# vislearn/esac

Hardware: NVIDIA H100
Metric: pose hypotheses scored/sec (640x480, 256 hyp x E experts) (higher is better)
Workload: dtype f32 (scoring) / f64 (P3P, refinement)

## Files before the change

esac_b200/csrc/capi.cu:

```cuda
#include <cuda_runtime.h>
#include <dlfcn.h>
#include <stdarg.h>
#include <stdio.h>
#include <stdlib.h>
#include <string.h>

#include <algorithm>
#include <exception>
#include <new>
#include <string>
#include <vector>
#include <thread>
#include <chrono>

#include "../../include/esac_b200.h"
#include "../../include/esac_b200_testhooks.h"
#include "esac_internal.h"
#include "esac_p3p_fast.cuh"
#include "esac_rng.cuh"

using namespace esacb200;

namespace {

// ... 225 lines not shown
    if (is_device_ptr(assign)) {
        pl.d_assign = (const long long*)assign;
        pl.assign_stride = stride;
    } else {
        std::vector<long long> tmp((size_t)P.M);
        for (int h = 0; h < P.M; ++h) tmp[h] = (long long)assign[(long long)h * stride];
        CK(abuf.ensure((size_t)P.M * 8));
        CK(cudaMemcpyAsync(abuf.p, tmp.data(), (size_t)P.M * 8, cudaMemcpyHostToDevice, copy_stream));
        pl.d_assign = abuf.as<long long>();
        pl.assign_stride = 1;
    }
    return 0;
}

void plan_launch(esacb200_ctx* ctx, Plan& pl) {
    const Problem& P = pl.P;
    int ppt = 8, hc = 64;
    const int want = 2 * 2 * ctx->sm_count;
    auto items = [&](int ppt_, int hc_) {
        int T = (P.N + score_tile_pixels(ppt_) - 1) / score_tile_pixels(ppt_);
        int nch = (P.M + hc_ - 1) / hc_ + (P.E > 1 ? P.E / 2 : 0);
        return (long long)T * nch;
    };
    if (items(8, 64) < want) { ppt = 4; hc = 32; }
    if (ppt == 4 && items(4, 32) < want) { ppt = 2; hc = 16; }
    if (ctx->score_ppt_opt == 2 || ctx->score_ppt_opt == 4 || ctx->score_ppt_opt == 8) ppt = ctx->score_ppt_opt;
    if (ctx->score_hc_opt > 0) hc = ctx->score_hc_opt < 64 ? ctx->score_hc_opt : 64;
    pl.ppt = ppt;
    pl.hc = hc;
    pl.T = (P.N + score_tile_pixels(ppt) - 1) / score_tile_pixels(ppt);
    const int max_chunks = (P.M + hc - 1) / hc + P.E;
    long long it = (long long)pl.T * max_chunks;
    pl.grid = (int)(it < 2ll * ctx->sm_count ? it : 2ll * ctx->sm_count);
    const int need_align = ppt >= 4 ? 4 : 2;
    pl.vec_ok = (P.N % need_align == 0) && (((uintptr_t)pl.d_coords) % (need_align * 4) == 0);
}

int plan_and_prep(esacb200_ctx* ctx, Plan& pl) {
    const Problem& P = pl.P;
    plan_launch(ctx, pl);
    CK(ctx->assign32.ensure((size_t)P.M * 4));
    CK(ctx->counts.ensure((size_t)P.E * 4));
    CK(ctx->offsets.ensure((size_t)(P.E + 1) * 4));
    CK(ctx->perm.ensure((size_t)P.M * 4));
    CK(ctx->slot_of.ensure((size_t)P.M * 4));
    CK(ctx->chunks.ensure((size_t)(P.M + P.E) * sizeof(ChunkDesc)));
    CK(ctx->scalars.ensure(S_COUNT * 4));
    CK(ctx->centres.ensure((size_t)P.E * 3 * 4));
    CK(ctx->poses.ensure((size_t)P.M * sizeof(Pose)));
    CK(ctx->poses_ref.ensure((size_t)P.M * sizeof(Pose)));
    CK(ctx->cells.ensure((size_t)P.M * 8 * 4));
    CK(ctx->tries.ensure((size_t)P.M * 4));
    CK(ctx->posepk.ensure((size_t)P.M * sizeof(PosePk)));
    CK(ctx->part.ensure((size_t)P.M * pl.T * 4));
    CK(ctx->scores.ensure((size_t)P.M * 8));
    CK(ctx->probs.ensure((size_t)P.M * 8));
    CK(ctx->stats.ensure(8 * 8));
    CK(ctx->contrib.ensure((size_t)P.M * 4));
    CK(ctx->out17.ensure(32 * 4));
    int* sc = ctx->scalars.as<int>();
    launch_prep(pl.d_coords, pl.d_assign, pl.assign_stride, P, pl.hc, ctx->assign32.as<int>(), ctx->counts.as<int>(),
                ctx->offsets.as<int>(), ctx->perm.as<int>(), ctx->slot_of.as<int>(), ctx->chunks.as<ChunkDesc>(),
                sc + S_NCHUNKS, sc + S_WORK, ctx->centres.as<float>(), sc + S_FLAGS, pl.split_e ? 1 : 3, ctx->stream);
    ctx->st.kernel_launches += 1;
    mark(ctx, EV_PREP);
    return 0;
}

int stage_inputs(esacb200_ctx* ctx, Plan& pl, const float* coords, const int64_t* assign, int64_t stride, bool allow_split = false) {
    int rc = upload_inputs(ctx, pl, coords, assign, stride, ctx->coords, ctx->assign64, ctx->stream, allow_split);
    if (rc) return rc;
    mark(ctx, EV_H2D);
    return plan_and_prep(ctx, pl);
}

constexpr int kSampleCap = 1 << 19;
constexpr int kSampleCapAcc = 1 << 15;

struct SampleSizes {
    int G, Mg;
    size_t per_group_ints, int_bytes, per_group_bytes, surv_bytes;
};
SampleSizes sample_sizes(const esacb200_ctx* ctx, const Plan& pl) {
    const Problem& P = pl.P;
    SampleSizes z;
    int G = pl.split_e ? 2 : ((ctx->sample_groups > 1 && ctx->aux_stream && P.M >= 64 && (P.N >= 65536 || P.M >= 1024)) ? ctx->sample_groups : 1);
    if (G > 2 && (!ctx->aux_more[0] || !ctx->aux_more[1] || P.M < 512)) G = 2;
    z.G = G;
    z.Mg = pl.split_e ? P.M : (P.M + G - 1) / G;
    z.per_group_ints = (size_t)2 * z.Mg + 8;
    z.int_bytes = ((size_t)P.M * 4 + G * z.per_group_ints) * 4 + 8;
    z.per_group_bytes = (size_t)kSampleCap * sizeof(int2) + (size_t)kSampleCapAcc * sizeof(Accepted);
    z.surv_bytes = G * z.per_group_bytes;
    return z;
}

int run_sample(esacb200_ctx* ctx, const Plan& pl, uint64_t seed) {
    const Problem& P = pl.P;
    const int cap = kSampleCap;
    const int cap_acc = kSampleCapAcc;
    const SampleSizes z = sample_sizes(ctx, pl);
    const int G = z.G, Mg = z.Mg;
    const size_t per_group_ints = z.per_group_ints, per_group_bytes = z.per_group_bytes;
    CK(ctx->smp_int.ensure(z.int_bytes));
    CK(ctx->smp_surv.ensure(z.surv_bytes));
    SampleState st[4];
    int* b = ctx->smp_int.as<int>() + 2 * (size_t)P.M;
    for (int g = 0; g < G; ++g) {
        st[g].best = ctx->smp_int.as<unsigned long long>();
        st[g].base = b;
        st[g].ovf = b + P.M;
        st[g].list = b + 2 * (size_t)P.M + g * per_group_ints;
        st[g].counters = st[g].list + 2 * (size_t)Mg;
        char* sb = (char*)ctx->smp_surv.p + g * per_group_bytes;
        st[g].surv = (int2*)sb;
        st[g].stage = (Accepted*)(sb + (size_t)cap * sizeof(int2));
        st[g].cap = cap;
        st[g].cap_acc = cap_acc;
        st[g].M = Mg;
    }
    CK(ctx->coords4.ensure((size_t)P.E * P.N * sizeof(float4)));
    unsigned long long* trace = nullptr;
    if (ctx->sample_trace) {
        CK(ctx->smp_trace.ensure(512 * 8));
        CK(cudaMemsetAsync(ctx->smp_trace.p, 0, 512 * 8, ctx->stream));
        trace = ctx->smp_trace.as<unsigned long long>();
        launch_trace_init(trace, 256, ctx->stream);
    }
    const cudaStream_t lane_streams[4] = {ctx->stream, ctx->aux_stream, ctx->aux_more[0], ctx->aux_more[1]};
    const cudaEvent_t lane_joins[4] = {nullptr, ctx->ev_join, ctx->ev_join_more[0], ctx->ev_join_more[1]};
    ctx->st.kernel_launches += launch_sample(pl.d_coords, ctx->coords4.as<float4>(), ctx->assign32.as<int>(), P, seed, ctx->max_tries,
                                             ctx->inj_M ? ctx->inject.as<int>() : nullptr, ctx->inj_T, st, G, ctx->sm_count,
                                             ctx->sample_prefilter, ctx->hyp_offset, ctx->hyp_stride, ctx->poses.as<Pose>(), ctx->cells.as<int>(),
                                             ctx->tries.as<int>(), lane_streams, ctx->ev_fork, lane_joins,
                                             pl.split_e, ctx->perm.as<int>(), ctx->offsets.as<int>(), ctx->ev_copied,
                                             ctx->sample_span0, ctx->sample_window, ctx->sample_waves, trace, ctx->sample_tail_boost);
    CK(cudaGetLastError());
    ctx->smp_groups_last = G;
    ctx->smp_Mg_last = Mg;
    if (pl.split_e) {
        int* sc = ctx->scalars.as<int>();
        launch_prep(pl.d_coords, pl.d_assign, pl.assign_stride, P, pl.hc, ctx->assign32.as<int>(), ctx->counts.as<int>(),
                    ctx->offsets.as<int>(), ctx->perm.as<int>(), ctx->slot_of.as<int>(), ctx->chunks.as<ChunkDesc>(),
                    sc + S_NCHUNKS, sc + S_WORK, ctx->centres.as<float>(), sc + S_FLAGS, 2, ctx->stream);
        ctx->st.kernel_launches += 1;
    }
    mark(ctx, EV_SAMPLE);
    return 0;
}

int run_score(esacb200_ctx* ctx, const Plan& pl) {
    const Problem& P = pl.P;
    int* sc = ctx->scalars.as<int>();
    launch_fold(ctx->poses.as<Pose>(), ctx->perm.as<int>(), ctx->assign32.as<int>(), ctx->centres.as<float>(), P,
                ctx->posepk.as<PosePk>(), ctx->stream);
    mark(ctx, EV_FOLD);
    ScoreArgs a;
    a.coords = pl.d_coords;
    a.centres = ctx->centres.as<float>();
    a.poses = ctx->posepk.as<PosePk>();
    a.chunks = ctx->chunks.as<ChunkDesc>();
    a.n_chunks = sc + S_NCHUNKS;
    a.work_counter = sc + S_WORK;
    a.part = ctx->part.as<float>();
    a.P = P;
    a.T = pl.T;
    a.hc = pl.hc;
    const float log2e = 1.4426950408889634f;
    a.k1 = P.beta * log2e;
    a.k0 = -P.beta * P.tau * log2e;
    a.vec_ok = pl.vec_ok;
    launch_score(a, pl.ppt, pl.grid, ctx->stream);
    mark(ctx, EV_SCORE);
    launch_select(ctx->part.as<float>(), ctx->slot_of.as<int>(), P, pl.T, ctx->scores.as<double>(), ctx->probs.as<double>(),
                  ctx->stats.as<double>(), sc + S_WINNER, ctx->contrib.as<int>(), sc + S_NCONTRIB, ctx->stream);
    mark(ctx, EV_SELECT);
    ctx->st.kernel_launches += 3;
    ctx->st.score_launches += 1;
    ctx->st.score_ppt = pl.ppt;
    ctx->st.score_grid = pl.grid;
    return 0;
}

int pick_group(esacb200_ctx* ctx, const Problem& P, int jobs_hint) {
    if (ctx->refine_group_opt > 0) return ctx->refine_group_opt < ctx->refine_coresident ? ctx->refine_group_opt : ctx->refine_coresident;
    const int words = (P.N + 31) / 32;
    int g = words / 10;
    if (g < 1) g = 1;
    int waves = jobs_hint >= 8 ? ctx->refine_jobs_per_group : 1;
    int concurrent = jobs_hint > 0 ? (jobs_hint + waves - 1) / waves : 1;
    int cap = ctx->refine_coresident / concurrent;
    if (waves > 1 && (cap < 1 || P.N / (cap < 1 ? 1 : cap) < 4096)) cap = ctx->refine_coresident / (jobs_hint > 0 ? jobs_hint : 1);
    if (cap < 1) cap = 1;
    if (g > cap) g = cap;
    return g;
}

struct RefineSizes {
    int n_groups, cache;
    size_t masks, rounds, scratch, n_flags, barrier, clist;
};
RefineSizes refine_sizes(const esacb200_ctx* ctx, const Problem& P, int max_jobs, int group) {
    RefineSizes z;
    const int words = (P.N + 31) / 32;
    int n_groups = ctx->refine_coresident / group;
    if (n_groups > max_jobs) n_groups = max_jobs;
    if (n_groups < 1) n_groups = 1;
    z.n_groups = n_groups;
    z.masks = (size_t)max_jobs * 2 * words * 4;
    z.rounds = (size_t)max_jobs * 2 * 4;
    z.scratch = refine_scratch_doubles(n_groups, group) * 8;
    z.n_flags = refine_flag_words(n_groups, group);
    z.barrier = (z.n_flags + 4) * 4;
    const int wpc = (words + group - 1) / group;
    z.cache = wpc <= refine_cache_words() ? 1 : 0;
    z.clist = (ctx->refine_compact && !z.cache && wpc <= refine_max_compact_words())
                  ? (size_t)n_groups * words * 32 * sizeof(unsigned short) : 0;
    return z;
}

int run_refine(esacb200_ctx* ctx, const Plan& pl, const Pose* in, Pose* out, const int* d_jobs, const int* d_njobs,
               int n_jobs_host, int max_jobs, int group) {
    const Problem& P = pl.P;
    const int words = (P.N + 31) / 32;
    const RefineSizes z = refine_sizes(ctx, P, max_jobs, group);
    const int n_groups = z.n_groups;
    CK(ctx->masks.ensure(z.masks));
    CK(ctx->rounds.ensure(z.rounds));
    CK(ctx->scratch.ensure(z.scratch));
    if (group > 1) CK(cudaMemsetAsync(ctx->scratch.p, 0, refine_scratch_doubles(n_groups, group) * 8, ctx->stream));
    const size_t n_flags = z.n_flags;
    CK(ctx->barrier.ensure(z.barrier));
    CK(cudaMemsetAsync(ctx->barrier.p, 0, z.barrier, ctx->stream));
    RefineArgs a;
    a.coords = pl.d_coords;
    a.centres = ctx->centres.as<float>();
    a.assign32 = ctx->assign32.as<int>();
    a.poses_in = in;
    a.poses_out = out;
    a.jobs = d_jobs;
    a.n_jobs = d_njobs;
    a.n_jobs_host = n_jobs_host;
    a.masks = ctx->masks.as<uint32_t>();
    a.mask_words = words;
    a.rounds = ctx->rounds.as<int>();
    a.scratch = ctx->scratch.as<double>();
    a.barrier = ctx->barrier.as<unsigned int>();
    a.job_counter = (int*)(ctx->barrier.as<unsigned int>() + n_flags);
    a.group = group;
    a.cache = z.cache;
    a.compact = ctx->refine_compact;
    a.pretest = ctx->refine_pretest;
    a.clist = nullptr;
    if (z.clist) {
        CK(ctx->clist.ensure(z.clist));
        a.clist = ctx->clist.as<unsigned short>();
    }
    a.prof = nullptr;
    if (ctx->refine_profile) {
        CK(ctx->prof.ensure(16 * 8));
        CK(cudaMemsetAsync(ctx->prof.p, 0, 16 * 8, ctx->stream));
        a.prof = ctx->prof.as<long long>();
    }
    a.P = P;
    a.max_ref_steps = ctx->max_ref_steps;
    launch_refine(a, n_groups, ctx->stream);
    CK(cudaGetLastError());
    ctx->st.kernel_launches += 1;
    ctx->st.refine_group = group;
    return 0;
}

uint64_t call_seed(esacb200_ctx* ctx) {
    uint64_t s = ctx->fixed_seed ? ctx->seed : mix64(ctx->seed + kGold * ctx->calls);
    if (ctx->calls == 0) s = ctx->seed;
    ++ctx->calls;
    return s;
}

int enqueue_forward_core(esacb200_ctx* ctx, const Plan& pl, float* d_out17) {
    const Problem& P = pl.P;
    int* sc = ctx->scalars.as<int>();
    const uint64_t seed = call_seed(ctx);
    int rc = run_sample(ctx, pl, seed);
    if (rc) return rc;
    rc = run_score(ctx, pl);
    if (rc) return rc;
    const int group = pick_group(ctx, P, 1);
    rc = run_refine(ctx, pl, ctx->poses.as<Pose>(), ctx->poses_ref.as<Pose>(), sc + S_WINNER, nullptr, 1, 1, group);
    if (rc) return rc;
    mark(ctx, EV_REFINE);
    launch_finish_forward(ctx->poses_ref.as<Pose>(), sc + S_WINNER, ctx->assign32.as<int>(), sc + S_FLAGS, d_out17, ctx->stream);
    ctx->st.kernel_launches += 1;
    return 0;
}

int reserve_forward_batch(esacb200_ctx* ctx, const std::vector<Plan>& plans, bool host_coords) {
    size_t part = 0, cbytes = 0, c4 = 0, sint = 0, ssurv = 0, masks = 0, rounds = 0, scratch = 0, barrier = 0, clist = 0;
    auto mx = [](size_t& a, size_t b) { if (b > a) a = b; };
    int M = 0, E = 0;
    for (Plan pl : plans) {
        plan_launch(ctx, pl);
        const Problem& P = pl.P;
        M = P.M; E = P.E;
        mx(part, (size_t)P.M * pl.T * 4);
        mx(cbytes, (size_t)P.E * 3 * P.N * sizeof(float));
        mx(c4, (size_t)P.E * P.N * sizeof(float4));
        const SampleSizes a = sample_sizes(ctx, pl);
        mx(sint, a.int_bytes);
        mx(ssurv, a.surv_bytes);
        const RefineSizes r = refine_sizes(ctx, P, 1, pick_group(ctx, P, 1));
        mx(masks, r.masks); mx(rounds, r.rounds); mx(scratch, r.scratch); mx(barrier, r.barrier); mx(clist, r.clist);
    }
    if (host_coords) {
        CK(ctx->coords.ensure(cbytes));
        CK(ctx->coords_alt.ensure(cbytes));
    }
    CK(ctx->assign64.ensure((size_t)M * 8));
    CK(ctx->assign64_alt.ensure((size_t)M * 8));
    CK(ctx->assign32.ensure((size_t)M * 4));
    CK(ctx->counts.ensure((size_t)E * 4));
    CK(ctx->offsets.ensure((size_t)(E + 1) * 4));
    CK(ctx->perm.ensure((size_t)M * 4));
// ... 1452 lines not shown
```

esac_b200/csrc/esac_internal.h:

```cpp
#pragma once
#include <cuda_runtime.h>
#include <stdint.h>

#include "esac_geom.cuh"

namespace esacb200 {

#ifdef __CUDACC__
template <int NV>
__device__ __forceinline__ double warp_reduce_scatter(const double (&v)[NV]) {
    static_assert(NV <= 32, "at most 32 values");
    const int lane = threadIdx.x & 31;
    double w[32];
#pragma unroll
    for (int i = 0; i < 32; ++i) w[i] = i < NV ? v[i] : 0.0;
#pragma unroll
    for (int o = 16; o >= 1; o >>= 1) {
        const bool up = (lane & o) != 0;
#pragma unroll
        for (int i = 0; i < o; ++i) {
            const double keep = up ? w[i + o] : w[i];
            const double send = up ? w[i] : w[i + o];
            w[i] = keep + __shfl_xor_sync(0xffffffffu, send, o);
        }
    }
    return w[0];
}

template <int THREADS, int NV>
__device__ __forceinline__ void block_sum_fixed(double (&v)[NV]) {
    __shared__ double warp_sum[NV][THREADS / 32];
#pragma unroll
    for (int i = 0; i < NV; ++i) {
#pragma unroll
        for (int o = 16; o > 0; o >>= 1) v[i] += __shfl_xor_sync(0xffffffffu, v[i], o);
    }
    __syncthreads();
    if ((threadIdx.x & 31) == 0) {
#pragma unroll
        for (int i = 0; i < NV; ++i) warp_sum[i][threadIdx.x >> 5] = v[i];
    }
    __syncthreads();
#pragma unroll
    for (int i = 0; i < NV; ++i) {
        double s = 0.;
        if (threadIdx.x == 0)
            for (int w = 0; w < THREADS / 32; ++w) s += warp_sum[i][w];
        v[i] = s;
    }
}

template <int THREADS, int NV>
__device__ __forceinline__ bool block_image_sum(double (&v)[NV], double* __restrict__ partial, unsigned* __restrict__ tickets,
                                                int b, unsigned blocks, size_t part0) {
    __shared__ bool last;
    block_sum_fixed<THREADS, NV>(v);
    if (threadIdx.x == 0) {
#pragma unroll
        for (int i = 0; i < NV; ++i) partial[(part0 + blockIdx.x) * NV + i] = v[i];
        __threadfence();
        last = atomicAdd(&tickets[b], 1u) == blocks - 1;
    }
    __syncthreads();
    if (!last) return false;
    __threadfence();
#pragma unroll
    for (int i = 0; i < NV; ++i) v[i] = 0.;
    for (unsigned k = threadIdx.x; k < blocks; k += THREADS) {
#pragma unroll
        for (int i = 0; i < NV; ++i) v[i] += __ldcg(&partial[(part0 + k) * NV + i]);
    }
    block_sum_fixed<THREADS, NV>(v);
    if (threadIdx.x == 0) tickets[b] = 0;
    return threadIdx.x == 0;
}
#endif

struct Problem {
    int E, H, W, N, M;
    int shiftX, shiftY, sub;
    float f, ppx, ppy;
    float tau, alpha, beta, max_reproj;
};

constexpr int kMaxChunk = 64;
struct ChunkDesc {
    int expert;
    int slot0;
    int count;
    int pad;
};

struct PosePk {
    float4 v[3];
};

struct ScoreArgs {
    const float* coords;
    const float* centres;
    const PosePk* poses;
    const ChunkDesc* chunks;
    const int* n_chunks;
    int* work_counter;
    float* part;
    Problem P;
    int T;
    int hc;
    float k1, k0;
    int vec_ok;
};

void launch_prep(const float* coords, const long long* assign, long long assign_stride, const Problem& P, int hc,
                 int* assign32, int* counts, int* offsets, int* perm, int* slot_of, ChunkDesc* chunks, int* n_chunks,
                 int* work_counter, float* centres, int* flags, int roles, cudaStream_t st);
void launch_fold(const Pose* poses, const int* perm, const int* assign32, const float* centres, const Problem& P,
                 PosePk* out, cudaStream_t st);
int score_tile_pixels(int ppt);
void launch_score(const ScoreArgs& a, int ppt, int grid, cudaStream_t st);
void launch_select(const float* part, const int* slot_of, const Problem& P, int T, double* scores, double* probs,
                   double* stats , int* winner, int* contrib,
                   int* n_contrib, cudaStream_t st);

void launch_rescale_probs(const double* scores, const Problem& P, double gmax, double gsum, double* probs, int* contrib,
                          int* n_contrib, cudaStream_t st);
void launch_rescale_probs_gathered(const double* scores, const Problem& P, const double* pairs, int world, double* norm_out,
                                   double* probs, int* contrib, int* n_contrib, cudaStream_t st);

struct Accepted {
    Pose pose;
    int cells[8];
};
struct SampleState {
    unsigned long long* best;
    Accepted* stage;
    int cap_acc;
    int* base;
    int* ovf;
    int* list;
    int2* surv;
    int cap;
    int* counters;
    int M;
};
int launch_sample(const float* coords, float4* coords4, const int* assign32, const Problem& P, uint64_t seed, int max_tries,
                  const int* injected, int inj_T, const SampleState* st, int n_lanes, int sm_count, int use_prefilter,
                  int hyp_offset, int hyp_stride, Pose* poses, int* cells, int* tries, const cudaStream_t* lanes,
                  cudaEvent_t ev_fork, const cudaEvent_t* ev_join, int split_e, const int* perm, const int* offsets,
                  const cudaEvent_t* ev_half, int span0, float window, int n_waves,
                  unsigned long long* trace, float tail_boost);
void launch_trace_init(unsigned long long* trace, int slots, cudaStream_t st);

struct RefineArgs {
    const float* coords;
    const float* centres;
    const int* assign32;
    const Pose* poses_in;
    Pose* poses_out;
    const int* jobs;
    const int* n_jobs;
    int n_jobs_host;
    uint32_t* masks;
    int mask_words;
    int* rounds;
    double* scratch;
    unsigned int* barrier;
    int* job_counter;
    int group;
    int cache;
    int compact;
    int pretest;
    unsigned short* clist;
    long long* prof;
    Problem P;
    int max_ref_steps;
};
void launch_refine(const RefineArgs& a, int n_groups, cudaStream_t st);
int refine_max_coresident_blocks(int sm_count);
int refine_cache_words();
int refine_max_compact_words();
size_t refine_scratch_doubles(int n_groups, int group);
size_t refine_flag_words(int n_groups, int group);
void launch_finish_forward(const Pose* poses, const int* winner, const int* assign32, const int* flags, float* out20,
                           cudaStream_t st);

void launch_pack_forward(const double* scores, const float* out20, int M, int M_pad, int expert_offset, int hyp_offset, int hyp_stride,
                         double* pack, cudaStream_t st);
constexpr int kPackTail = 21;
void launch_select_gathered(const double* gathered, int world, int M_pad, float* out20, cudaStream_t st);

int assign_max_experts();
void launch_assign(const float* weights, int B, int E, int M, int keep_top, int single, uint64_t seed, int64_t* out_assign,
                   float* out_hist, int* flags, cudaStream_t stream);

int reproj_blocks_per_image(int N);
struct ReprojImage {
    const float* coords;
    float* grads;
    int N, W;
    int b;
    int blocks;
    long long part0;
};
bool reproj_vec_ok(const float* coords, const float* grads, int N, int W);
constexpr int kReprojImgFloats = 20;
void launch_reproj(bool vec, const ReprojImage* recs, int n, int max_blocks, const float* img, float sub, float cut,
                   float max_err, float min_depth, double* partial, unsigned* tickets, double* losses, cudaStream_t stream);

struct CoordImage {
    const float* pred;
    const float* gt;
    float* grads;
    int Np, Ng;
    int Wp, Wg;
    int H, W;
    int N;
    int b;
    int blocks;
    int pad;
    long long part0;
};
bool coord_image(CoordImage& r, int Hp, int Wp, int Hg, int Wg);
void launch_coord_loss(bool vec, int pass, bool grad, const CoordImage* recs, int n, int max_blocks, float cut,
                       unsigned* counts, double* partial, unsigned* tickets, double* losses, long long* out_counts,
                       cudaStream_t stream);

struct BwdArgs {
    const float* coords;
    float* grads;
    const int* assign32;
    const int* perm;
    const int* counts;
    const int* offsets;
    const Pose* init;
    const Pose* ref;
    const int* cells;
    const double* probs;
    const int* contrib;
    const int* n_contrib;
    const int* job_of;
    const uint32_t* masks;
    int mask_words;
    const int* rounds;
    double* losses;
    double* out_loss;
    double* red;
    void* hyp_grad;
    float gt[16];
    float wRot, wTrans, cut;
    Problem P;
    const double* expected_override;
};
void launch_backward(const BwdArgs& a, int max_jobs, int sm_count, cudaStream_t st);
void launch_backward_losses(const BwdArgs& a, cudaStream_t st);
void launch_add_inplace(float* dst, const float* src, size_t n, cudaStream_t st);
void launch_expert_flags(const int* contrib, const int* n_contrib, const int* assign32, int E, int* flags, cudaStream_t st);
size_t bwd_hypgrad_bytes();
int bwd_red_vals();
int bwd_tiles(int N);

}
```

esac_b200/csrc/score.cu:

```cuda
#include <atomic>

#include "esac_internal.h"

namespace esacb200 {

constexpr int kScoreThreads = 256;

__global__ void __launch_bounds__(1024) prep_kernel(const float* __restrict__ coords, const long long* __restrict__ assign,
                                                    long long stride, Problem P, int hc, int* assign32, int* counts,
                                                    int* offsets, int* perm, int* slot_of, ChunkDesc* chunks,
                                                    int* n_chunks, int* work_counter, float* centres, int* flags,
                                                    int with_assign) {
    const int tid = threadIdx.x;
    if (with_assign && blockIdx.x == 0) {
        if (tid == 0) { *work_counter = 0; flags[0] = 0; }
        for (int e = tid; e < P.E; e += blockDim.x) counts[e] = 0;
        __syncthreads();
        for (int h = tid; h < P.M; h += blockDim.x) {
            long long e = assign[(long long)h * stride];
            if (e < 0 || e >= P.E) { flags[0] = 1; e = 0; }
            assign32[h] = (int)e;
            atomicAdd(&counts[(int)e], 1);
        }
        __syncthreads();
        if (tid == 0) {
            int acc = 0, nc = 0;
            for (int e = 0; e < P.E; ++e) {
                offsets[e] = acc;
                for (int s = 0; s < counts[e]; s += hc) {
                    ChunkDesc c;
                    c.expert = e; c.slot0 = acc + s; c.count = min(hc, counts[e] - s); c.pad = 0;
                    chunks[nc++] = c;
                }
                acc += counts[e];
            }
            offsets[P.E] = acc;
            *n_chunks = nc;
        }
        __syncthreads();
        {
            const int lane = tid & 31, warp = tid >> 5, nwarps = blockDim.x >> 5;
            for (int e = warp; e < P.E; e += nwarps) {
                if (counts[e] == 0) continue;
                int pos = offsets[e];
                for (int b = 0; b < P.M; b += 32) {
                    const int h = b + lane;
                    const bool mine = h < P.M && assign32[h] == e;
                    const unsigned m = __ballot_sync(0xffffffffu, mine);
                    if (mine) {
                        const int q = pos + __popc(m & ((1u << lane) - 1u));
                        perm[q] = h;
                        slot_of[h] = q;
                    }
                    pos += __popc(m);
                }
            }
        }
    } else {
        const int e = blockIdx.x - with_assign;
        const float* pl = coords + (size_t)e * 3 * P.N;
        const int ns = min(P.N, 4096);
        const int step = max(1, P.N / ns);
        float sx = 0, sy = 0, sz = 0, cnt = 0;
        for (int i = tid; i < ns; i += blockDim.x) {
            int p = min(i * step, P.N - 1);
            float x = pl[p], y = pl[P.N + p], z = pl[2 * P.N + p];
            if (isfinite(x) && isfinite(y) && isfinite(z) && fabsf(x) < 1e18f && fabsf(y) < 1e18f && fabsf(z) < 1e18f) {
                sx += x; sy += y; sz += z; cnt += 1;
            }
        }
        __shared__ float red[4][32];
        for (int o = 16; o; o >>= 1) {
            sx += __shfl_xor_sync(0xffffffffu, sx, o);
            sy += __shfl_xor_sync(0xffffffffu, sy, o);
            sz += __shfl_xor_sync(0xffffffffu, sz, o);
            cnt += __shfl_xor_sync(0xffffffffu, cnt, o);
        }
        if ((tid & 31) == 0) { red[0][tid >> 5] = sx; red[1][tid >> 5] = sy; red[2][tid >> 5] = sz; red[3][tid >> 5] = cnt; }
        __syncthreads();
        if (tid == 0) {
            float a = 0, b = 0, c = 0, n = 0;
            for (int w = 0; w < (int)(blockDim.x >> 5); ++w) { a += red[0][w]; b += red[1][w]; c += red[2][w]; n += red[3][w]; }
            float inv = n > 0 ? 1.f / n : 0.f;
            centres[e * 3 + 0] = a * inv; centres[e * 3 + 1] = b * inv; centres[e * 3 + 2] = c * inv;
        }
    }
}

void launch_prep(const float* coords, const long long* assign, long long assign_stride, const Problem& P, int hc,
                 int* assign32, int* counts, int* offsets, int* perm, int* slot_of, ChunkDesc* chunks, int* n_chunks,
                 int* work_counter, float* centres, int* flags, int roles, cudaStream_t st) {
    const int with_assign = roles & 1, n_centres = (roles & 2) ? P.E : 0;
    if (with_assign + n_centres == 0) return;
    prep_kernel<<<with_assign + n_centres, 1024, 0, st>>>(coords, assign, assign_stride, P, hc, assign32, counts, offsets, perm,
                                                          slot_of, chunks, n_chunks, work_counter, centres, flags, with_assign);
}

__global__ void fold_kernel(const Pose* __restrict__ poses, const int* __restrict__ perm, const int* __restrict__ assign32,
                            const float* __restrict__ centres, Problem P, PosePk* __restrict__ out) {
    int s = blockIdx.x * blockDim.x + threadIdx.x;
    if (s >= P.M) return;
    int h = perm[s];
    int e = assign32[h];
    Pose p = poses[h];
    double R[9];
    rodrigues_v2m(p.r, R, nullptr);
    double c[3] = {(double)centres[e * 3], (double)centres[e * 3 + 1], (double)centres[e * 3 + 2]};
    double f = (double)P.f;
    float A[12];
    for (int r = 0; r < 3; ++r) {
        double sc = r < 2 ? f : 1.0;
        double b = R[r * 3] * c[0] + R[r * 3 + 1] * c[1] + R[r * 3 + 2] * c[2] + p.t[r];
        A[r * 4 + 0] = (float)(sc * R[r * 3 + 0]);
        A[r * 4 + 1] = (float)(sc * R[r * 3 + 1]);
        A[r * 4 + 2] = (float)(sc * R[r * 3 + 2]);
        A[r * 4 + 3] = (float)(sc * b);
    }
    PosePk pk;
    for (int r = 0; r < 3; ++r) pk.v[r] = make_float4(A[r * 4 + 0], A[r * 4 + 1], A[r * 4 + 2], A[r * 4 + 3]);
    out[s] = pk;
}

void launch_fold(const Pose* poses, const int* perm, const int* assign32, const float* centres, const Problem& P,
                 PosePk* out, cudaStream_t st) {
    fold_kernel<<<(P.M + 127) / 128, 128, 0, st>>>(poses, perm, assign32, centres, P, out);
}

__device__ __forceinline__ float mufu_rsq(float x) {
    float y;
    asm("rsqrt.approx.ftz.f32 %0, %1;" : "=f"(y) : "f"(x));
    return y;
}
__device__ __forceinline__ float mufu_ex2(float x) {
    float y;
    asm("ex2.approx.ftz.f32 %0, %1;" : "=f"(y) : "f"(x));
    return y;
}
__device__ __forceinline__ float mufu_rcp(float x) {
    float y;
    asm("rcp.approx.ftz.f32 %0, %1;" : "=f"(y) : "f"(x));
    return y;
}

template <int PPT, bool TAIL>
__device__ __forceinline__ void score_item(const ScoreArgs& a, const ChunkDesc cd, const int tile, const float4* sPose,
                                           float (*sWarp)[kMaxChunk], const float* tileX = nullptr,
                                           const float* tileY = nullptr, const float* tileZ = nullptr) {
    constexpr int NP = PPT / 2;
    constexpr int GV = PPT >= 4 ? 4 : 2;
    constexpr int NG = PPT / GV;
    constexpr int TP = kScoreThreads * PPT;
    const int tid = threadIdx.x, lane = tid & 31, warp = tid >> 5;
    const Problem& P = a.P;
    const float* pl = a.coords + (size_t)cd.expert * 3 * P.N;
    const float cX = a.centres[cd.expert * 3], cY = a.centres[cd.expert * 3 + 1], cZ = a.centres[cd.expert * 3 + 2];

    float2 X[NP], Y[NP], Z[NP], A[NP], B[NP], V[NP];
#pragma unroll
    for (int g = 0; g < NG; ++g) {
        const int p0 = tile * TP + g * (kScoreThreads * GV) + tid * GV;
        float x[GV], y[GV], z[GV];
        if (tileX) {
            const int o = g * (kScoreThreads * GV) + tid * GV;
            if (!TAIL) {
                if constexpr (GV == 4) {
                    const float4 vx = *(const float4*)(tileX + o), vy = *(const float4*)(tileY + o), vz = *(const float4*)(tileZ + o);
                    x[0] = vx.x; x[1] = vx.y; x[GV - 2] = vx.z; x[GV - 1] = vx.w;
                    y[0] = vy.x; y[1] = vy.y; y[GV - 2] = vy.z; y[GV - 1] = vy.w;
                    z[0] = vz.x; z[1] = vz.y; z[GV - 2] = vz.z; z[GV - 1] = vz.w;
                } else {
                    const float2 vx = *(const float2*)(tileX + o), vy = *(const float2*)(tileY + o), vz = *(const float2*)(tileZ + o);
                    x[0] = vx.x; x[1] = vx.y; y[0] = vy.x; y[1] = vy.y; z[0] = vz.x; z[1] = vz.y;
                }
            } else {
                const int last = P.N - 1 - tile * TP;
#pragma unroll
                for (int i = 0; i < GV; ++i) {
                    const int q = min(o + i, last);
                    x[i] = tileX[q]; y[i] = tileY[q]; z[i] = tileZ[q];
                }
            }
        } else if (a.vec_ok && p0 + GV <= P.N) {
            if constexpr (GV == 4) {
                float4 vx = __ldg((const float4*)(pl + p0));
                float4 vy = __ldg((const float4*)(pl + P.N + p0));
                float4 vz = __ldg((const float4*)(pl + 2 * (size_t)P.N + p0));
                x[0] = vx.x; x[1] = vx.y; x[GV - 2] = vx.z; x[GV - 1] = vx.w;
                y[0] = vy.x; y[1] = vy.y; y[GV - 2] = vy.z; y[GV - 1] = vy.w;
                z[0] = vz.x; z[1] = vz.y; z[GV - 2] = vz.z; z[GV - 1] = vz.w;
            } else {
                float2 vx = __ldg((const float2*)(pl + p0));
                float2 vy = __ldg((const float2*)(pl + P.N + p0));
                float2 vz = __ldg((const float2*)(pl + 2 * (size_t)P.N + p0));
                x[0] = vx.x; x[1] = vx.y; y[0] = vy.x; y[1] = vy.y; z[0] = vz.x; z[1] = vz.y;
            }
        } else {
#pragma unroll
            for (int i = 0; i < GV; ++i) {
                int p = min(p0 + i, P.N - 1);
                x[i] = __ldg(pl + p); y[i] = __ldg(pl + P.N + p); z[i] = __ldg(pl + 2 * (size_t)P.N + p);
            }
        }
        float aa[GV], bb[GV], vv[GV];
#pragma unroll
        for (int i = 0; i < GV; ++i) {
            int p = p0 + i;
            int py = p / P.W, px = p - py * P.W;
            aa[i] = P.ppx - (float)(px * P.sub + P.sub / 2 - P.shiftX);
            bb[i] = P.ppy - (float)(py * P.sub + P.sub / 2 - P.shiftY);
            vv[i] = (p < P.N) ? 1.f : 0.f;
            x[i] -= cX; y[i] -= cY; z[i] -= cZ;
        }
#pragma unroll
        for (int i = 0; i < GV / 2; ++i) {
            const int j = g * (GV / 2) + i;
            X[j] = make_float2(x[2 * i], x[2 * i + 1]);
            Y[j] = make_float2(y[2 * i], y[2 * i + 1]);
            Z[j] = make_float2(z[2 * i], z[2 * i + 1]);
            A[j] = make_float2(aa[2 * i], aa[2 * i + 1]);
            B[j] = make_float2(bb[2 * i], bb[2 * i + 1]);
            V[j] = make_float2(vv[2 * i], vv[2 * i + 1]);
        }
    }
    const float2 k1 = make_float2(a.k1, a.k1), k0 = make_float2(a.k0, a.k0);
    const float2 one = make_float2(1.f, 1.f), tiny = make_float2(1e-30f, 1e-30f);
    const float mr = P.max_reproj;

    auto one_hyp = [&](int hl) -> float {
        const float4* q = sPose + hl * 3;
        const float4 r0 = q[0], r1 = q[1], r2 = q[2];
        const float2 a00 = make_float2(r0.x, r0.x), a01 = make_float2(r0.y, r0.y), a02 = make_float2(r0.z, r0.z), b0 = make_float2(r0.w, r0.w);
        const float2 a10 = make_float2(r1.x, r1.x), a11 = make_float2(r1.y, r1.y), a12 = make_float2(r1.z, r1.z), b1 = make_float2(r1.w, r1.w);
        const float2 a20 = make_float2(r2.x, r2.x), a21 = make_float2(r2.y, r2.y), a22 = make_float2(r2.z, r2.z), b2 = make_float2(r2.w, r2.w);
        float2 acc = make_float2(0.f, 0.f);
#pragma unroll
        for (int j = 0; j < NP; ++j) {
            float2 xc = ffma2(a00, X[j], ffma2(a01, Y[j], ffma2(a02, Z[j], b0)));
            float2 yc = ffma2(a10, X[j], ffma2(a11, Y[j], ffma2(a12, Z[j], b1)));
            float2 zc = ffma2(a20, X[j], ffma2(a21, Y[j], ffma2(a22, Z[j], b2)));
            float2 pu = ffma2(A[j], zc, xc);
            float2 pv = ffma2(B[j], zc, yc);
            float2 num = ffma2(pu, pu, ffma2(pv, pv, tiny));
            float2 m = fmul2(fmul2(zc, zc), num);
            float2 rs = make_float2(mufu_rsq(m.x), mufu_rsq(m.y));
            float2 err = fmul2(num, rs);
            err.x = fminf(err.x, mr);
            err.y = fminf(err.y, mr);
            float2 t = ffma2(err, k1, k0);
            float2 ex = make_float2(mufu_ex2(t.x), mufu_ex2(t.y));
            float2 den = fadd2(ex, one);
            float2 w = make_float2(mufu_rcp(den.x), mufu_rcp(den.y));
            if (TAIL) acc = ffma2(w, V[j], acc);
            else acc = fadd2(acc, w);
        }
        return acc.x + acc.y;
    };

    int hl = 0;
    for (; hl + 4 <= cd.count; hl += 4) {
        const float v0 = one_hyp(hl), v1 = one_hyp(hl + 1), v2 = one_hyp(hl + 2), v3 = one_hyp(hl + 3);
        const bool hi16 = lane & 16, hi8 = lane & 8;
        float k0_ = hi16 ? v2 : v0, k1_ = hi16 ? v3 : v1;
        float s0_ = hi16 ? v0 : v2, s1_ = hi16 ? v1 : v3;
        k0_ += __shfl_xor_sync(0xffffffffu, s0_, 16);
        k1_ += __shfl_xor_sync(0xffffffffu, s1_, 16);
        float c = hi8 ? k1_ : k0_;
        const float d = hi8 ? k0_ : k1_;
        c += __shfl_xor_sync(0xffffffffu, d, 8);
        c += __shfl_xor_sync(0xffffffffu, c, 4);
        c += __shfl_xor_sync(0xffffffffu, c, 2);
        c += __shfl_xor_sync(0xffffffffu, c, 1);
        if ((lane & 7) == 0) sWarp[warp][hl + (lane >> 3)] = c;
    }
    for (; hl < cd.count; ++hl) {
        float s = one_hyp(hl);
#pragma unroll
        for (int o = 16; o; o >>= 1) s += __shfl_xor_sync(0xffffffffu, s, o);
        if (lane == 0) sWarp[warp][hl] = s;
    }
    __syncthreads();
    if (tid < cd.count) {
        float s = 0.f;
#pragma unroll
        for (int w = 0; w < kScoreThreads / 32; ++w) s += sWarp[w][tid];
        a.part[(size_t)(cd.slot0 + tid) * a.T + tile] = s;
    }
}

template <int PPT>
__global__ void __launch_bounds__(kScoreThreads, 2) score_kernel(const __grid_constant__ ScoreArgs a) {
    __shared__ float4 sPose[kMaxChunk * 3];
    __shared__ float sWarp[kScoreThreads / 32][kMaxChunk];
    __shared__ int sItem;
    constexpr int TP = kScoreThreads * PPT;
    const int tid = threadIdx.x;
    const int n_items = *a.n_chunks * a.T;
    const bool ragged = (a.P.N % TP) != 0;
    for (;;) {
        if (tid == 0) sItem = atomicAdd(a.work_counter, 1);
        __syncthreads();
        const int item = sItem;
        if (item >= n_items) break;
        const int chunk = item / a.T, tile = item - chunk * a.T;
        const ChunkDesc cd = a.chunks[chunk];
        const float4* src = (const float4*)(a.poses + cd.slot0);
        for (int i = tid; i < cd.count * 3; i += kScoreThreads) sPose[i] = src[i];
        __syncthreads();
        if (ragged && tile == a.T - 1) score_item<PPT, true>(a, cd, tile, sPose, sWarp);
        else score_item<PPT, false>(a, cd, tile, sPose, sWarp);
        __syncthreads();
    }
}

__device__ __forceinline__ uint32_t smem_u32(const void* p) { return (uint32_t)__cvta_generic_to_shared(p); }
__device__ __forceinline__ void mbar_init(uint64_t* bar, int count) {
    asm volatile("mbarrier.init.shared::cta.b64 [%0], %1;" ::"r"(smem_u32(bar)), "r"(count));
}
__device__ __forceinline__ void mbar_expect_tx(uint64_t* bar, uint32_t bytes) {
    asm volatile("mbarrier.arrive.expect_tx.shared::cta.b64 _, [%0], %1;" ::"r"(smem_u32(bar)), "r"(bytes) : "memory");
}
__device__ __forceinline__ void mbar_wait(uint64_t* bar, uint32_t parity) {
    asm volatile(
        "{\n\t.reg .pred p;\n\t"
        "WAIT_%=:\n\t"
        "mbarrier.try_wait.parity.shared::cta.b64 p, [%0], %1;\n\t"
        "@p bra DONE_%=;\n\t"
        "bra WAIT_%=;\n\t"
        "DONE_%=:\n\t}" ::"r"(smem_u32(bar)), "r"(parity) : "memory");
}
__device__ __forceinline__ void tma_bulk_g2s(void* dst, const void* src, uint32_t bytes, uint64_t* bar) {
    asm volatile("cp.async.bulk.shared::cluster.global.mbarrier::complete_tx::bytes [%0], [%1], %2, [%3];" ::"r"(smem_u32(dst)),
                 "l"(src), "r"(bytes), "r"(smem_u32(bar))
                 : "memory");
}

template <int PPT>
__global__ void __launch_bounds__(kScoreThreads, 2) score_kernel_tma(const __grid_constant__ ScoreArgs a) {
    constexpr int TP = kScoreThreads * PPT;
    extern __shared__ __align__(128) float sTile[];
    __shared__ float4 sPose[kMaxChunk * 3];
    __shared__ float sWarp[kScoreThreads / 32][kMaxChunk];
    __shared__ __align__(8) uint64_t sBar[2];
    __shared__ int sItem[2];
    const int tid = threadIdx.x;
    const int n_items = *a.n_chunks * a.T;
    const bool ragged = (a.P.N % TP) != 0;

    auto issue = [&](int item, int stage) {
        const int chunk = item / a.T, tile = item - chunk * a.T;
        const int e = a.chunks[chunk].expert;
        const int cells = min(TP, a.P.N - tile * TP);
        const uint32_t bytes = (uint32_t)cells * 4u;
        const float* src = a.coords + (size_t)e * 3 * a.P.N + (size_t)tile * TP;
        float* dst = sTile + (size_t)stage * 3 * TP;
        mbar_expect_tx(&sBar[stage], 3u * bytes);
        tma_bulk_g2s(dst, src, bytes, &sBar[stage]);
        tma_bulk_g2s(dst + TP, src + a.P.N, bytes, &sBar[stage]);
        tma_bulk_g2s(dst + 2 * TP, src + 2 * (size_t)a.P.N, bytes, &sBar[stage]);
    };

    if (tid == 0) {
        mbar_init(&sBar[0], 1);
        mbar_init(&sBar[1], 1);
        asm volatile("fence.mbarrier_init.release.cluster;" ::: "memory");
        const int first = atomicAdd(a.work_counter, 1);
        sItem[0] = first;
        if (first < n_items) issue(first, 0);
    }
    __syncthreads();
    uint32_t phase[2] = {0u, 0u};
    for (int it = 0;; ++it) {
        const int stage = it & 1;
        const int item = sItem[stage];
        if (item >= n_items) break;
        if (tid == 0) {
            const int nxt = atomicAdd(a.work_counter, 1);
            sItem[stage ^ 1] = nxt;
            if (nxt < n_items) {
                asm volatile("fence.proxy.async.shared::cta;" ::: "memory");
                issue(nxt, stage ^ 1);
            }
        }
        const int chunk = item / a.T, tile = item - chunk * a.T;
        const ChunkDesc cd = a.chunks[chunk];
        const float4* src = (const float4*)(a.poses + cd.slot0);
        for (int i = tid; i < cd.count * 3; i += kScoreThreads) sPose[i] = src[i];
        mbar_wait(&sBar[stage], phase[stage]);
        phase[stage] ^= 1u;
        __syncthreads();
        const float* tx = sTile + (size_t)stage * 3 * TP;
        if (ragged && tile == a.T - 1) score_item<PPT, true>(a, cd, tile, sPose, sWarp, tx, tx + TP, tx + 2 * TP);
        else score_item<PPT, false>(a, cd, tile, sPose, sWarp, tx, tx + TP, tx + 2 * TP);
        __syncthreads();
    }
}

int score_tile_pixels(int ppt) { return kScoreThreads * ppt; }

constexpr int kMaxDevices = 64;

void launch_score(const ScoreArgs& a, int ppt, int grid, cudaStream_t st) {
    if (a.vec_ok && ppt >= 4) {
        const size_t smem = (size_t)2 * 3 * kScoreThreads * ppt * sizeof(float);
        static std::atomic<unsigned char> attr_set[kMaxDevices][2];
        int dev = 0;
        cudaGetDevice(&dev);
        const int which = ppt == 8 ? 0 : 1;
        const bool known = dev >= 0 && dev < kMaxDevices;
        if (!known || !attr_set[dev][which].load(std::memory_order_acquire)) {
            if (ppt == 8) cudaFuncSetAttribute(score_kernel_tma<8>, cudaFuncAttributeMaxDynamicSharedMemorySize, (int)smem);
            else cudaFuncSetAttribute(score_kernel_tma<4>, cudaFuncAttributeMaxDynamicSharedMemorySize, (int)smem);
            if (known) attr_set[dev][which].store(1, std::memory_order_release);
        }
        if (ppt == 8) score_kernel_tma<8><<<grid, kScoreThreads, smem, st>>>(a);
        else score_kernel_tma<4><<<grid, kScoreThreads, smem, st>>>(a);
        return;
    }
    if (ppt == 8) score_kernel<8><<<grid, kScoreThreads, 0, st>>>(a);
    else if (ppt == 4) score_kernel<4><<<grid, kScoreThreads, 0, st>>>(a);
    else score_kernel<2><<<grid, kScoreThreads, 0, st>>>(a);
}

__global__ void __launch_bounds__(256) finish_scores_kernel(const float* __restrict__ part, const int* __restrict__ slot_of,
                                                            Problem P, int T, double* scores) {
    const int lane = threadIdx.x & 31;
    const int h = (blockIdx.x * blockDim.x + threadIdx.x) >> 5;
    if (h >= P.M) return;
    const float facf = P.alpha / (float)P.W / (float)P.H;
    const float* row = part + (size_t)slot_of[h] * T;
    double s = 0;
    for (int t = lane; t < T; t += 32) s += (double)row[t];
    for (int o = 16; o; o >>= 1) s += __shfl_xor_sync(0xffffffffu, s, o);
    if (lane == 0) scores[h] = s * (double)facf;
}

__global__ void __launch_bounds__(1024) select_kernel(const float* __restrict__ part, const int* __restrict__ slot_of,
                                                      Problem P, int T, double* scores, double* probs, double* stats,
                                                      int* winner, int* contrib, int* n_contrib) {
    __shared__ double sred[32];
    __shared__ int sidx[32];
    const int tid = threadIdx.x, lane = tid & 31, warp = tid >> 5, nw = blockDim.x >> 5;
    (void)part; (void)slot_of; (void)T;
    double mx = -1e300;
    for (int h = tid; h < P.M; h += blockDim.x) mx = fmax(mx, scores[h]);
    for (int o = 16; o; o >>= 1) mx = fmax(mx, __shfl_xor_sync(0xffffffffu, mx, o));
    if (lane == 0) sred[warp] = mx;
    __syncthreads();
    mx = sred[0];
    for (int w = 1; w < nw; ++w) mx = fmax(mx, sred[w]);
    __syncthreads();
    double sum = 0;
    for (int h = tid; h < P.M; h += blockDim.x) {
        double e = exp(scores[h] - mx);
        probs[h] = e;
        sum += e;
    }
    for (int o = 16; o; o >>= 1) sum += __shfl_xor_sync(0xffffffffu, sum, o);
    if (lane == 0) sred[warp] = sum;
    __syncthreads();
    sum = 0;
    for (int w = 0; w < nw; ++w) sum += sred[w];
    __syncthreads();
    double ent = 0, best = -1;
    int bi = 0x7fffffff;
    for (int h = tid; h < P.M; h += blockDim.x) {
        double p = probs[h] / sum;
        probs[h] = p;
        if (p > 0) ent -= p * log2(p);
        if (!(p < kEps) && (p > best)) { best = p; bi = h; }
    }
    for (int o = 16; o; o >>= 1) {
        ent += __shfl_xor_sync(0xffffffffu, ent, o);
        double ob = __shfl_xor_sync(0xffffffffu, best, o);
        int oi = __shfl_xor_sync(0xffffffffu, bi, o);
        if (ob > best || (ob == best && oi < bi)) { best = ob; bi = oi; }
    }
    if (lane == 0) { sred[warp] = best; sidx[warp] = bi; }
    __syncthreads();
    __shared__ double sent[32];
    if (lane == 0) sent[warp] = ent;
    __syncthreads();
    __shared__ int swc[32];
    __shared__ int srun;
    if (tid == 0) {
        double b = -1; int i = 0x7fffffff; double en = 0;
        for (int w = 0; w < nw; ++w) {
            en += sent[w];
            if (sred[w] > b || (sred[w] == b && sidx[w] < i)) { b = sred[w]; i = sidx[w]; }
        }
        if (i == 0x7fffffff) i = 0;
        *winner = i;
        stats[0] = en; stats[1] = (double)i;
        stats[5] = mx; stats[6] = sum;
        srun = 0;
    }
    __syncthreads();
    for (int b = 0; b < P.M; b += blockDim.x) {
        const int h = b + tid;
        const bool flag = h < P.M && !(probs[h] < kProbThresh);
        const unsigned m = __ballot_sync(0xffffffffu, flag);
        if (lane == 0) swc[warp] = __popc(m);
        __syncthreads();
        int off = srun;
        for (int w = 0; w < warp; ++w) off += swc[w];
        if (flag) contrib[off + __popc(m & ((1u << lane) - 1u))] = h;
        __syncthreads();
        if (tid == 0) { int t = 0; for (int w = 0; w < nw; ++w) t += swc[w]; srun += t; }
        __syncthreads();
    }
    if (tid == 0) { *n_contrib = srun; stats[2] = (double)srun; }
}

void launch_select(const float* part, const int* slot_of, const Problem& P, int T, double* scores, double* probs,
                   double* stats, int* winner, int* contrib, int* n_contrib, cudaStream_t st) {
    finish_scores_kernel<<<(P.M * 32 + 255) / 256, 256, 0, st>>>(part, slot_of, P, T, scores);
    select_kernel<<<1, 1024, 0, st>>>(part, slot_of, P, T, scores, probs, stats, winner, contrib, n_contrib);
}


__global__ void __launch_bounds__(1024) rescale_probs_kernel(const double* __restrict__ scores, Problem P, double gmax, double gsum,
                                                             double* probs, int* contrib, int* n_contrib) {
    __shared__ int swc[32];
    __shared__ int srun;
    const int tid = threadIdx.x, lane = tid & 31, warp = tid >> 5, nw = blockDim.x >> 5;
    if (tid == 0) srun = 0;
    __syncthreads();
    for (int b = 0; b < P.M; b += blockDim.x) {
        const int h = b + tid;
        bool flag = false;
        if (h < P.M) {
            const double p = exp(scores[h] - gmax) / gsum;
            probs[h] = p;
            flag = !(p < kProbThresh);
        }
        const unsigned m = __ballot_sync(0xffffffffu, flag);
        if (lane == 0) swc[warp] = __popc(m);
        __syncthreads();
        int off = srun;
        for (int w = 0; w < warp; ++w) off += swc[w];
        if (flag) contrib[off + __popc(m & ((1u << lane) - 1u))] = h;
        __syncthreads();
        if (tid == 0) { int t = 0; for (int w = 0; w < nw; ++w) t += swc[w]; srun += t; }
        __syncthreads();
    }
    if (tid == 0) *n_contrib = srun;
}

void launch_rescale_probs(const double* scores, const Problem& P, double gmax, double gsum, double* probs, int* contrib,
                          int* n_contrib, cudaStream_t st) {
    rescale_probs_kernel<<<1, 1024, 0, st>>>(scores, P, gmax, gsum, probs, contrib, n_contrib);
}

__global__ void __launch_bounds__(1024) rescale_probs_gathered_kernel(const double* __restrict__ scores, Problem P,
                                                                      const double* __restrict__ pairs, int world, double* norm_out,
                                                                      double* probs, int* contrib, int* n_contrib) {
    __shared__ int swc[32];
    __shared__ int srun;
    __shared__ double snorm[2];
    const int tid = threadIdx.x, lane = tid & 31, warp = tid >> 5, nw = blockDim.x >> 5;
    if (tid == 0) {
        srun = 0;
        double gmax = -1e300;
        for (int r = 0; r < world; ++r) gmax = fmax(gmax, pairs[2 * r]);
        double gsum = 0;
        for (int r = 0; r < world; ++r) gsum += pairs[2 * r + 1] * exp(pairs[2 * r] - gmax);
        snorm[0] = gmax; snorm[1] = gsum;
        if (norm_out) { norm_out[0] = gmax; norm_out[1] = gsum; }
    }
    __syncthreads();
    const double gmax = snorm[0], gsum = snorm[1];
    for (int b = 0; b < P.M; b += blockDim.x) {
        const int h = b + tid;
        bool flag = false;
// ... 25 lines not shown
```

Before: 914,100.

## Fold soft-inlier scale into poses and share one reciprocal per pixel pair

```diff
diff --git a/esac_b200/csrc/capi.cu b/esac_b200/csrc/capi.cu
--- a/esac_b200/csrc/capi.cu
+++ b/esac_b200/csrc/capi.cu
@@ -401,10 +401,11 @@
 int run_score(esacb200_ctx* ctx, const Plan& pl) {
     const Problem& P = pl.P;
     int* sc = ctx->scalars.as<int>();
+    ScoreArgs a;
+    score_constants(P, a);
     launch_fold(ctx->poses.as<Pose>(), ctx->perm.as<int>(), ctx->assign32.as<int>(), ctx->centres.as<float>(), P,
-                ctx->posepk.as<PosePk>(), ctx->stream);
+                a.fold ? a.k1 : 1.f, ctx->posepk.as<PosePk>(), ctx->stream);
     mark(ctx, EV_FOLD);
-    ScoreArgs a;
     a.coords = pl.d_coords;
     a.centres = ctx->centres.as<float>();
     a.poses = ctx->posepk.as<PosePk>();
@@ -415,9 +416,6 @@
     a.P = P;
     a.T = pl.T;
     a.hc = pl.hc;
-    const float log2e = 1.4426950408889634f;
-    a.k1 = P.beta * log2e;
-    a.k0 = -P.beta * P.tau * log2e;
     a.vec_ok = pl.vec_ok;
     launch_score(a, pl.ppt, pl.grid, ctx->stream);
     mark(ctx, EV_SCORE);
diff --git a/esac_b200/csrc/esac_internal.h b/esac_b200/csrc/esac_internal.h
--- a/esac_b200/csrc/esac_internal.h
+++ b/esac_b200/csrc/esac_internal.h
@@ -107,6 +107,9 @@
     int T;
     int hc;
     float k1, k0;
+    float tmax;
+    float tiny;
+    int fold;
     int vec_ok;
 };
 
@@ -114,8 +117,9 @@
                  int* assign32, int* counts, int* offsets, int* perm, int* slot_of, ChunkDesc* chunks, int* n_chunks,
                  int* work_counter, float* centres, int* flags, int roles, cudaStream_t st);
 void launch_fold(const Pose* poses, const int* perm, const int* assign32, const float* centres, const Problem& P,
-                 PosePk* out, cudaStream_t st);
+                 float kf, PosePk* out, cudaStream_t st);
 int score_tile_pixels(int ppt);
+void score_constants(const Problem& P, ScoreArgs& a);
 void launch_score(const ScoreArgs& a, int ppt, int grid, cudaStream_t st);
 void launch_select(const float* part, const int* slot_of, const Problem& P, int T, double* scores, double* probs,
                    double* stats , int* winner, int* contrib,
diff --git a/esac_b200/csrc/score.cu b/esac_b200/csrc/score.cu
--- a/esac_b200/csrc/score.cu
+++ b/esac_b200/csrc/score.cu
@@ -5,6 +5,7 @@
 namespace esacb200 {
 
 constexpr int kScoreThreads = 256;
+constexpr int kScorePairShift = 32;
 
 __global__ void __launch_bounds__(1024) prep_kernel(const float* __restrict__ coords, const long long* __restrict__ assign,
                                                     long long stride, Problem P, int hc, int* assign32, int* counts,
@@ -97,7 +98,7 @@
 }
 
 __global__ void fold_kernel(const Pose* __restrict__ poses, const int* __restrict__ perm, const int* __restrict__ assign32,
-                            const float* __restrict__ centres, Problem P, PosePk* __restrict__ out) {
+                            const float* __restrict__ centres, Problem P, float kf, PosePk* __restrict__ out) {
     int s = blockIdx.x * blockDim.x + threadIdx.x;
     if (s >= P.M) return;
     int h = perm[s];
@@ -106,7 +107,7 @@
     double R[9];
     rodrigues_v2m(p.r, R, nullptr);
     double c[3] = {(double)centres[e * 3], (double)centres[e * 3 + 1], (double)centres[e * 3 + 2]};
-    double f = (double)P.f;
+    const double f = (double)P.f * (double)kf;
     float A[12];
     for (int r = 0; r < 3; ++r) {
         double sc = r < 2 ? f : 1.0;
@@ -122,8 +123,23 @@
 }
 
 void launch_fold(const Pose* poses, const int* perm, const int* assign32, const float* centres, const Problem& P,
-                 PosePk* out, cudaStream_t st) {
-    fold_kernel<<<(P.M + 127) / 128, 128, 0, st>>>(poses, perm, assign32, centres, P, out);
+                 float kf, PosePk* out, cudaStream_t st) {
+    fold_kernel<<<(P.M + 127) / 128, 128, 0, st>>>(poses, perm, assign32, centres, P, kf, out);
+}
+
+void score_constants(const Problem& P, ScoreArgs& a) {
+    const float log2e = 1.4426950408889634f;
+    a.k1 = P.beta * log2e;
+    a.k0 = -P.beta * P.tau * log2e;
+    const float k0s = a.k0 - (float)kScorePairShift;
+    a.tmax = fmaf(P.max_reproj, a.k1, k0s);
+    a.fold = a.k1 >= 1e-3f && std::isfinite(a.k1) && std::isfinite(k0s) && a.tmax <= 63.f;
+    if (a.fold) {
+        a.k0 = k0s;
+        a.tiny = 1e-30f * a.k1 * a.k1;
+    } else {
+        a.tiny = 1e-30f;
+    }
 }
 
 __device__ __forceinline__ float mufu_rsq(float x) {
@@ -142,7 +158,7 @@
     return y;
 }
 
-template <int PPT, bool TAIL>
+template <int PPT, bool TAIL, bool FOLD>
 __device__ __forceinline__ void score_item(const ScoreArgs& a, const ChunkDesc cd, const int tile, const float4* sPose,
                                            float (*sWarp)[kMaxChunk], const float* tileX = nullptr,
                                            const float* tileY = nullptr, const float* tileZ = nullptr) {
@@ -208,6 +224,7 @@
             int py = p / P.W, px = p - py * P.W;
             aa[i] = P.ppx - (float)(px * P.sub + P.sub / 2 - P.shiftX);
             bb[i] = P.ppy - (float)(py * P.sub + P.sub / 2 - P.shiftY);
+            if (FOLD) { aa[i] = __fmul_rn(aa[i], a.k1); bb[i] = __fmul_rn(bb[i], a.k1); }
             vv[i] = (p < P.N) ? 1.f : 0.f;
             x[i] -= cX; y[i] -= cY; z[i] -= cZ;
         }
@@ -223,8 +240,9 @@
         }
     }
     const float2 k1 = make_float2(a.k1, a.k1), k0 = make_float2(a.k0, a.k0);
-    const float2 one = make_float2(1.f, 1.f), tiny = make_float2(1e-30f, 1e-30f);
-    const float mr = P.max_reproj;
+    const float2 one = make_float2(1.f, 1.f), tiny = make_float2(a.tiny, a.tiny);
+    const float mr = FOLD ? a.tmax : P.max_reproj;
+    const float d0 = 1.f / (float)(1ull << kScorePairShift);
 
     auto one_hyp = [&](int hl) -> float {
         const float4* q = sPose + hl * 3;
@@ -243,6 +261,20 @@
             float2 num = ffma2(pu, pu, ffma2(pv, pv, tiny));
             float2 m = fmul2(fmul2(zc, zc), num);
             float2 rs = make_float2(mufu_rsq(m.x), mufu_rsq(m.y));
+            if (FOLD) {
+                const float ta = fminf(__fmaf_rn(num.x, rs.x, k0.x), mr), tb = fminf(__fmaf_rn(num.y, rs.y, k0.x), mr);
+                const float da = __fadd_rn(mufu_ex2(ta), d0);
+                float db = __fadd_rn(mufu_ex2(tb), d0), ds;
+                if (TAIL) {
+                    const bool vb = V[j].y != 0.f;
+                    ds = __fmul_rn(vb ? __fadd_rn(da, db) : da, V[j].x);
+                    db = vb ? db : da;
+                } else {
+                    ds = __fadd_rn(da, db);
+                }
+                acc.x = __fmaf_rn(ds, mufu_rcp(__fmul_rn(da, db)), acc.x);
+                continue;
+            }
             float2 err = fmul2(num, rs);
             err.x = fminf(err.x, mr);
             err.y = fminf(err.y, mr);
@@ -253,7 +285,7 @@
             if (TAIL) acc = ffma2(w, V[j], acc);
             else acc = fadd2(acc, w);
         }
-        return acc.x + acc.y;
+        return FOLD ? acc.x : acc.x + acc.y;
     };
 
     int hl = 0;
@@ -283,11 +315,12 @@
         float s = 0.f;
 #pragma unroll
         for (int w = 0; w < kScoreThreads / 32; ++w) s += sWarp[w][tid];
+        if (FOLD) s *= 1.f / (float)(1ull << kScorePairShift);
         a.part[(size_t)(cd.slot0 + tid) * a.T + tile] = s;
     }
 }
 
-template <int PPT>
+template <int PPT, bool FOLD>
 __global__ void __launch_bounds__(kScoreThreads, 2) score_kernel(const __grid_constant__ ScoreArgs a) {
     __shared__ float4 sPose[kMaxChunk * 3];
     __shared__ float sWarp[kScoreThreads / 32][kMaxChunk];
@@ -306,8 +339,8 @@
         const float4* src = (const float4*)(a.poses + cd.slot0);
         for (int i = tid; i < cd.count * 3; i += kScoreThreads) sPose[i] = src[i];
         __syncthreads();
-        if (ragged && tile == a.T - 1) score_item<PPT, true>(a, cd, tile, sPose, sWarp);
-        else score_item<PPT, false>(a, cd, tile, sPose, sWarp);
+        if (ragged && tile == a.T - 1) score_item<PPT, true, FOLD>(a, cd, tile, sPose, sWarp);
+        else score_item<PPT, false, FOLD>(a, cd, tile, sPose, sWarp);
         __syncthreads();
     }
 }
@@ -334,7 +367,7 @@
                  : "memory");
 }
 
-template <int PPT>
+template <int PPT, bool FOLD>
 __global__ void __launch_bounds__(kScoreThreads, 2) score_kernel_tma(const __grid_constant__ ScoreArgs a) {
     constexpr int TP = kScoreThreads * PPT;
     extern __shared__ __align__(128) float sTile[];
@@ -389,8 +422,8 @@
         phase[stage] ^= 1u;
         __syncthreads();
         const float* tx = sTile + (size_t)stage * 3 * TP;
-        if (ragged && tile == a.T - 1) score_item<PPT, true>(a, cd, tile, sPose, sWarp, tx, tx + TP, tx + 2 * TP);
-        else score_item<PPT, false>(a, cd, tile, sPose, sWarp, tx, tx + TP, tx + 2 * TP);
+        if (ragged && tile == a.T - 1) score_item<PPT, true, FOLD>(a, cd, tile, sPose, sWarp, tx, tx + TP, tx + 2 * TP);
+        else score_item<PPT, false, FOLD>(a, cd, tile, sPose, sWarp, tx, tx + TP, tx + 2 * TP);
         __syncthreads();
     }
 }
@@ -399,7 +432,8 @@
 
 constexpr int kMaxDevices = 64;
 
-void launch_score(const ScoreArgs& a, int ppt, int grid, cudaStream_t st) {
+template <bool FOLD>
+void launch_score_t(const ScoreArgs& a, int ppt, int grid, cudaStream_t st) {
     if (a.vec_ok && ppt >= 4) {
         const size_t smem = (size_t)2 * 3 * kScoreThreads * ppt * sizeof(float);
         static std::atomic<unsigned char> attr_set[kMaxDevices][2];
@@ -408,17 +442,22 @@
         const int which = ppt == 8 ? 0 : 1;
         const bool known = dev >= 0 && dev < kMaxDevices;
         if (!known || !attr_set[dev][which].load(std::memory_order_acquire)) {
-            if (ppt == 8) cudaFuncSetAttribute(score_kernel_tma<8>, cudaFuncAttributeMaxDynamicSharedMemorySize, (int)smem);
-            else cudaFuncSetAttribute(score_kernel_tma<4>, cudaFuncAttributeMaxDynamicSharedMemorySize, (int)smem);
+            if (ppt == 8) cudaFuncSetAttribute(score_kernel_tma<8, FOLD>, cudaFuncAttributeMaxDynamicSharedMemorySize, (int)smem);
+            else cudaFuncSetAttribute(score_kernel_tma<4, FOLD>, cudaFuncAttributeMaxDynamicSharedMemorySize, (int)smem);
             if (known) attr_set[dev][which].store(1, std::memory_order_release);
         }
-        if (ppt == 8) score_kernel_tma<8><<<grid, kScoreThreads, smem, st>>>(a);
-        else score_kernel_tma<4><<<grid, kScoreThreads, smem, st>>>(a);
+        if (ppt == 8) score_kernel_tma<8, FOLD><<<grid, kScoreThreads, smem, st>>>(a);
+        else score_kernel_tma<4, FOLD><<<grid, kScoreThreads, smem, st>>>(a);
         return;
     }
-    if (ppt == 8) score_kernel<8><<<grid, kScoreThreads, 0, st>>>(a);
-    else if (ppt == 4) score_kernel<4><<<grid, kScoreThreads, 0, st>>>(a);
-    else score_kernel<2><<<grid, kScoreThreads, 0, st>>>(a);
+    if (ppt == 8) score_kernel<8, FOLD><<<grid, kScoreThreads, 0, st>>>(a);
+    else if (ppt == 4) score_kernel<4, FOLD><<<grid, kScoreThreads, 0, st>>>(a);
+    else score_kernel<2, FOLD><<<grid, kScoreThreads, 0, st>>>(a);
+}
+
+void launch_score(const ScoreArgs& a, int ppt, int grid, cudaStream_t st) {
+    if (a.fold) launch_score_t<true>(a, ppt, grid, st);
+    else launch_score_t<false>(a, ppt, grid, st);
 }
 
 __global__ void __launch_bounds__(256) finish_scores_kernel(const float* __restrict__ part, const int* __restrict__ slot_of,
```

Result: faster. 945,800 (median of 6 runs) (+3.5%).
